# 959AI994/Multi-Gate-VAE

Measured on AMD Instinct MI355X. Metric: circuit-graphs/sec (train step), AIG-64k batch=64 per GPU, higher is better.
Workload: dtype f32 storage; dense products as bf16x3 split-precision MFMA, fp32 accumulate; 1 GPU; cfg2: DG_AE --type aig, 64 x 65536-node synthetic levelised DAGs per GPU (N=4194304, E=6558720, 120 levels), H=64, 4+4 rounds, layernorm, weights [1,4,4], negatives sampled; step includes the 7-scalar metrics copy (pinned, read one step behind); global_batch=64, parallelism=dp1

## Files before the change

### include/mgvae_hip.h

```cpp
#ifndef MGVAE_HIP_H
#define MGVAE_HIP_H
#include <stdint.h>
#ifdef __cplusplus
extern "C" {
#endif

#ifndef MGV_OK
#define MGV_OK 0
#define MGV_EINVAL (-1)
#define MGV_EUNSUPPORTED (-2)
#endif

int mgv_abi_version(void);

int mgv_struct_stage_fwd(int H, int64_t N, const float* h_in, const int32_t* nbr_ptr, const int32_t* nbr_idx,
                         const uint8_t* xcls, const float* xtab, int C, const float* Wc, const float* bc,
                         const float* Whh, const float* bhh, const float* ln_w, const float* ln_b, float ln_eps,
                         float* h_out, void* stream);
int mgv_struct_stage_bwd(int H, int64_t N, const float* h_in, const int32_t* nbr_ptr, const int32_t* nbr_idx,
                         const uint8_t* xcls, const float* xtab, int C, const float* Wc, const float* WcT,
                         const float* bc, const float* Whh, const float* WhhT, const float* bhh,
                         const float* ln_w, const float* ln_b, float ln_eps, const float* gy_direct,
                         const float* gy_agg, float* g_direct_out, float* g_agg_out, float* dWc, float* dbc,
                         float* dWhh, float* dbhh, float* dxtab, float* dln_w, float* dln_b, void* stream);
// ... 104 lines not shown
                          const float* gh, const float* h_prev, float* d_gh, float* g_hprev, void* stream);

int mgv_attn_pool_fwd(int W, int64_t N, const int32_t* in_ptr, const int32_t* in_src, const float* x, const float* u,
                      float* zbar, float* mstat, float* inv, void* stream);
int mgv_attn_pool_bwd(int W, int64_t N, const int32_t* in_ptr, const int32_t* in_src, const float* x, const float* u,
                      const float* zbar, const float* mstat, const float* inv, const float* dzbar, float* dx, float* du,
                      void* stream);

int mgv_sweep_pull_heavy(int H, int K, const int32_t* nodes, const int32_t* node_seg_ptr, int S, const int32_t* seg_e0,
                         const int32_t* seg_e1, const int32_t* out_dst, const int32_t* out_slot, const uint8_t* gslot,
                         const float* alpha, const float* dsc, const float* dzb, const float* attn_u, float* partial_ws,
                         float* ghs, void* stream);

int mgv_edge_dot_fwd(int H, int64_t E, const float* s, const float* t, int ld, const int64_t* src,
                     const int64_t* dst, int sigmoid, float* out, void* stream);
int mgv_edge_dot_bwd(int H, int64_t E, const float* s, const float* t, int ld, const int64_t* src,
                     const int64_t* dst, int sigmoid, const float* gout, float* ds, float* dt, void* stream);
int mgv_recon_loss_fwd(int H, const float* s, const float* t, int ld, const int64_t* pos_src, const int64_t* pos_dst,
                       int64_t Epos, const int64_t* neg_src, const int64_t* neg_dst, int64_t Eneg,
                       double* sums, uint64_t* counts, int32_t* pred_bin, double* workspace, int64_t workspace_doubles,
                       void* stream);
int mgv_recon_loss_bwd(int H, int64_t N, const float* s, const float* t, int ld, const int64_t* pos_src, const int64_t* pos_dst,
                       int64_t Epos, const int32_t* pos_out_ptr, const int32_t* pos_out_dst, const int32_t* pos_in_ptr,
                       const int32_t* pos_in_src, const int64_t* neg_src, const int64_t* neg_dst, int64_t Eneg,
                       const float* gscale, float* ds, float* dt, void* stream);
int mgv_recon_loss_bwd_csr(int H, int64_t N, const float* s, const float* t, int ld, const int32_t* pos_out_ptr,
                           const int32_t* pos_out_dst, const int32_t* pos_in_ptr, const int32_t* pos_in_src, int64_t Epos,
                           const int32_t* neg_out_ptr, const int32_t* neg_out_dst, const int32_t* neg_in_ptr,
                           const int32_t* neg_in_src, int64_t Eneg, const float* gscale, float* ds, float* dt,
                           int skip_pos_longer_than , void* stream);
int mgv_recon_heavy_lists(int H, const float* s, const float* t, int ld, int64_t Epos, const float* gscale, int K,
                          const int32_t* nodes, const int32_t* node_seg_ptr, int S, const int32_t* seg_node, const int32_t* seg_e0,
                          const int32_t* seg_e1, const int32_t* list, int which, float* partial_ws, float* out, void* stream);
int mgv_link_keys(int H, const float* s, const float* t, int ld, const int64_t* pos_src, const int64_t* pos_dst, int64_t P,
                  const int64_t* neg_src, const int64_t* neg_dst, int64_t Q, uint32_t* keys, float* scores, int32_t* status,
                  void* stream);
int mgv_link_rank_work_ints(int64_t n);
int mgv_link_rank(int64_t n, int64_t P, const uint32_t* sorted_keys, const int32_t* order, double* out, int32_t* work,
                  int64_t work_ints, void* stream);
int mgv_neg_sample(int64_t N, int64_t E, uint64_t seed, const int32_t* pos_out_ptr, const int32_t* pos_out_dst,
                   int64_t* neg_src, int64_t* neg_dst, int32_t* cnt_out, int32_t* cnt_in, int32_t* rank_out, int32_t* rank_in,
                   void* stream);
int mgv_neg_bucket(int64_t E, const int64_t* neg_src, const int64_t* neg_dst, const int32_t* out_ptr, const int32_t* in_ptr,
                   const int32_t* rank_out, const int32_t* rank_in, int64_t* srt_src, int64_t* srt_dst, int32_t* out_dst, int32_t* in_src,
                   void* stream);

int mgv_func_loss_fwd(int H, int64_t P, const float* hf, const int64_t* pair_a, const int64_t* pair_b,
                      const float* tt, float eps, float* dis, double* ws, double* workspace, int64_t workspace_doubles,
                      void* stream);
int mgv_func_loss_bwd_csr(int H, int64_t N, int64_t P, const float* hf, const int64_t* pair_a, const int64_t* pair_b, const float* tt_sim,
                          const float* dis, float eps, const double* workspace8, const float* grad_loss, const int32_t* a_ptr,
                          const int32_t* a_pair, const int32_t* b_ptr, const int32_t* b_pair, const float* add, float* dhf, void* stream);
int mgv_func_loss_bwd(int H, int64_t P, const float* hf, const int64_t* pair_a, const int64_t* pair_b,
                      const float* tt, const float* dis, float eps, const double* ws, const float* gscale,
                      float* dhf, void* stream);

int mgv_reparam_fwd(int64_t n, const float* mu, const float* logstd, const float* eps, uint64_t seed,
                    float* eps_out, float* z, double* klsum, void* stream);
int mgv_reparam_bwd(int64_t n, const float* mu, const float* logstd, const float* eps, const float* gz,
                    const float* gkl, float klcoef, float* dmu, float* dlogstd, void* stream);
int mgv_confusion(int64_t n, const int32_t* pred_bin, const int32_t* gt_bin, uint64_t* counts, void* stream);

int mgv_sum_workspace_doubles(void);
int mgv_colstats(int64_t N, int C, const float* Y, int ld, double* sums, double* workspace, int64_t workspace_doubles, void* stream);
int mgv_bn_act_fwd(int64_t N, int C, const float* Y, const float* mean, const float* invstd, const float* gamma,
                   const float* beta, float p_drop, uint64_t seed, float* A, void* stream);
// ... 87 lines not shown
```

### multi-gate-vae_amd/csrc/losses.hip

```cpp
#include "mgv_common.h"
#include "mgv_slab.h"
#include "../../include/mgvae_hip.h"

namespace mgv {

__device__ __forceinline__ void atomic_add4(float* p, const float4& v) {
    atomicAdd(p + 0, v.x); atomicAdd(p + 1, v.y); atomicAdd(p + 2, v.z); atomicAdd(p + 3, v.w);
}

__device__ __forceinline__ double block_sum_d(double v, double* red) {
    const int tid = threadIdx.x;
    __syncthreads();
    red[tid] = v;
    __syncthreads();
    for (int s = kThreads / 2; s > 0; s >>= 1) {
        if (tid < s) red[tid] += red[tid + s];
        __syncthreads();
    }
    return red[0];
}

template <int H, bool BWD>
__global__ __launch_bounds__(kThreads) void k_edge_dot(int64_t E, const float* s, const float* t, int ld,
                                                       const int64_t* src, const int64_t* dst, int sigmoid,
// ... 50 lines not shown
        if (ok) {
            u = pos ? a.psrc[e] : a.nsrc[e - a.Ep];
            v = pos ? a.pdst[e] : a.ndst[e - a.Ep];
            x = ld4(a.s + u * a.ld + 4 * lr);
            y = ld4(a.t + v * a.ld + 4 * lr);
        }
        const float val = group_sum<LPR>(dot4(x, y));
        const float p = sigmoidf_(val);
        if (!BWD) {
            if (ok && lr == 0) {
                const bool hit = p > 0.5f;
                if (pos) { lp -= logf(p + 1e-15f); tp += hit; fn += !hit; }
                else     { ln -= logf((1.0f - p) + 1e-15f); fp += hit; tn += !hit; }
                if (a.pred_bin) a.pred_bin[e] = hit ? 1 : 0;
            }
        } else if (ok) {
            const float dp = p * (1.0f - p);
            const float c = pos ? -wpos * dp / (p + 1e-15f) : wneg * dp / ((1.0f - p) + 1e-15f);
            atomic_add4(a.ds + u * a.ld + 4 * lr, scale4(c, y));
            atomic_add4(a.dt + v * a.ld + 4 * lr, scale4(c, x));
        }
    }
    if (!BWD) {
        const double sp = block_sum_d((double)lp, red);
        const double sn = block_sum_d((double)ln, red);
        const double c0 = block_sum_d((double)tp, red), c1 = block_sum_d((double)fp, red);
        const double c2 = block_sum_d((double)tn, red), c3 = block_sum_d((double)fn, red);
        if (threadIdx.x == 0) {
            a.slab[2 * blockIdx.x + 0] = sp; a.slab[2 * blockIdx.x + 1] = sn;
            atomicAdd(a.cnt + 0, (unsigned long long)c0); atomicAdd(a.cnt + 1, (unsigned long long)c1);
            atomicAdd(a.cnt + 2, (unsigned long long)c2); atomicAdd(a.cnt + 3, (unsigned long long)c3);
        }
    }
}

template <int H>
__global__ __launch_bounds__(kThreads) void k_recon_bwd_pull(int64_t N, const float* s, const float* t, int ld,
                                                             const int32_t* out_ptr, const int32_t* out_dst,
                                                             const int32_t* in_ptr, const int32_t* in_src, int64_t Ep,
                                                             const float* gscale, float* ds, float* dt) {
    constexpr int LPR = H / 4, RPB = kThreads / LPR;
    const int lr = threadIdx.x % LPR, slot = threadIdx.x / LPR;
    const float w = -(*gscale) / (float)Ep;
    for (int64_t n0 = (int64_t)blockIdx.x * RPB; n0 < N; n0 += (int64_t)gridDim.x * RPB) {
        const int64_t u = n0 + slot;
        if (u >= N) continue;
        const float4 su = ld4(s + u * ld + 4 * lr), tu = ld4(t + u * ld + 4 * lr);
        float4 gs = zero4(), gt = zero4();
        for (int e = out_ptr[u]; e < out_ptr[u + 1]; ++e) {
            const float4 tv = ld4(t + (int64_t)out_dst[e] * ld + 4 * lr);
            const float p = sigmoidf_(group_sum<LPR>(dot4(su, tv)));
            gs = fma4(w * p * (1.0f - p) / (p + 1e-15f), tv, gs);
        }
        for (int e = in_ptr[u]; e < in_ptr[u + 1]; ++e) {
            const float4 sv = ld4(s + (int64_t)in_src[e] * ld + 4 * lr);
            const float p = sigmoidf_(group_sum<LPR>(dot4(sv, tu)));
            gt = fma4(w * p * (1.0f - p) / (p + 1e-15f), sv, gt);
        }
        float* pds = ds + u * ld + 4 * lr;
        float* pdt = dt + u * ld + 4 * lr;
        st4(pds, add4(ld4(pds), gs));
        st4(pdt, add4(ld4(pdt), gt));
    }
}

template <int H>
// ... 281 lines not shown
        dmu[i] = g + gk * (-2.0f * m);
        dls[i] = g * eps[i] * sd + gk * (2.0f - 2.0f * sd * sd);
    }
}

__global__ __launch_bounds__(kThreads) void k_confusion(int64_t n, const int32_t* pred, const int32_t* gt, unsigned long long* cnt) {
    __shared__ double red[kThreads];
    unsigned int tp = 0, fp = 0, tn = 0, fn = 0;
    for (int64_t i = (int64_t)blockIdx.x * kThreads + threadIdx.x; i < n; i += (int64_t)gridDim.x * kThreads) {
        const int p = pred[i], g = gt[i];
        tp += (p == 1) & (g == 1); fp += (p == 1) & (g == 0); tn += (p == 0) & (g == 0); fn += (p == 0) & (g == 1);
    }
    const double c0 = block_sum_d((double)tp, red), c1 = block_sum_d((double)fp, red);
    const double c2 = block_sum_d((double)tn, red), c3 = block_sum_d((double)fn, red);
    if (threadIdx.x == 0) {
        atomicAdd(cnt + 0, (unsigned long long)c0); atomicAdd(cnt + 1, (unsigned long long)c1);
        atomicAdd(cnt + 2, (unsigned long long)c2); atomicAdd(cnt + 3, (unsigned long long)c3);
    }
}

inline int items_grid(int64_t items, int per_block) { return grid_for((items + per_block - 1) / per_block, 8); }

}

#define MGV_DISPATCH_H(H, CALL)                      \
    switch (H) {                                     \
        case 16: { constexpr int HH = 16; CALL; } break;  \
        case 32: { constexpr int HH = 32; CALL; } break;  \
        case 64: { constexpr int HH = 64; CALL; } break;  \
        case 128: { constexpr int HH = 128; CALL; } break; \
        default: return MGV_EUNSUPPORTED;            \
    }

extern "C" int mgv_edge_dot_fwd(int H, int64_t E, const float* s, const float* t, int ld, const int64_t* src,
                                const int64_t* dst, int sigmoid, float* out, void* stream) {
    MGV_CHECK_ARG(E >= 0 && s && t && out && ld >= H && ld % 4 == 0);
    if (E == 0) return MGV_OK;
    MGV_CHECK_ARG(src && dst);
    hipStream_t st = static_cast<hipStream_t>(stream);
    MGV_DISPATCH_H(H, hipLaunchKernelGGL((mgv::k_edge_dot<HH, false>), dim3(mgv::items_grid(E, mgv::kThreads / (HH / 4))), dim3(mgv::kThreads), 0, st,
                                         E, s, t, ld, src, dst, sigmoid, out, nullptr, nullptr, nullptr));
    MGV_LAUNCH_RET();
}

extern "C" int mgv_edge_dot_bwd(int H, int64_t E, const float* s, const float* t, int ld, const int64_t* src,
                                const int64_t* dst, int sigmoid, const float* gout, float* ds, float* dt, void* stream) {
    MGV_CHECK_ARG(E >= 0 && s && t && gout && ds && dt && ld >= H && ld % 4 == 0);
    if (E == 0) return MGV_OK;
    MGV_CHECK_ARG(src && dst);
    hipStream_t st = static_cast<hipStream_t>(stream);
    MGV_DISPATCH_H(H, hipLaunchKernelGGL((mgv::k_edge_dot<HH, true>), dim3(mgv::items_grid(E, mgv::kThreads / (HH / 4))), dim3(mgv::kThreads), 0, st,
                                         E, s, t, ld, src, dst, sigmoid, nullptr, gout, ds, dt));
    MGV_LAUNCH_RET();
}

extern "C" int mgv_recon_loss_fwd(int H, const float* s, const float* t, int ld, const int64_t* pos_src, const int64_t* pos_dst,
                                  int64_t Epos, const int64_t* neg_src, const int64_t* neg_dst, int64_t Eneg,
                                  double* sums, uint64_t* counts, int32_t* pred_bin, double* workspace, int64_t workspace_doubles,
                                  void* stream) {
    MGV_CHECK_ARG(s && t && sums && counts && Epos >= 0 && Eneg >= 0 && ld >= H && ld % 4 == 0);
    MGV_CHECK_ARG((Epos == 0 || (pos_src && pos_dst)) && (Eneg == 0 || (neg_src && neg_dst)));
    if (Epos + Eneg == 0) return MGV_OK;
    mgv::ReconArgs a{};
    a.s = s; a.t = t; a.ld = ld; a.psrc = pos_src; a.pdst = pos_dst; a.Ep = Epos; a.nsrc = neg_src; a.ndst = neg_dst; a.En = Eneg;
    a.sums = sums; a.cnt = reinterpret_cast<unsigned long long*>(counts); a.pred_bin = pred_bin;
    hipStream_t st = static_cast<hipStream_t>(stream);
    int grid = 0;
    MGV_DISPATCH_H(H, grid = mgv::items_grid(Epos + Eneg, mgv::kThreads / (HH / 4)));
    MGV_CHECK_ARG(workspace && workspace_doubles >= 2 * (int64_t)grid);
    a.slab = workspace;
    MGV_DISPATCH_H(H, hipLaunchKernelGGL((mgv::k_recon<HH, false>), dim3(grid), dim3(mgv::kThreads), 0, st, a));
    mgv::launch_slab_sum<double, double>(workspace, grid, 2, 2, sums, st);
    MGV_LAUNCH_RET();
}

extern "C" int mgv_recon_loss_bwd(int H, int64_t N, const float* s, const float* t, int ld, const int64_t* pos_src, const int64_t* pos_dst,
                                  int64_t Epos, const int32_t* pos_out_ptr, const int32_t* pos_out_dst, const int32_t* pos_in_ptr,
                                  const int32_t* pos_in_src, const int64_t* neg_src, const int64_t* neg_dst, int64_t Eneg,
                                  const float* gscale, float* ds, float* dt, void* stream) {
    MGV_CHECK_ARG(s && t && gscale && ds && dt && Epos >= 0 && Eneg >= 0 && N >= 0 && ld >= H && ld % 4 == 0);
    MGV_CHECK_ARG((Epos == 0 || (pos_src && pos_dst)) && (Eneg == 0 || (neg_src && neg_dst)));
    const bool pull = pos_out_ptr != nullptr;
    MGV_CHECK_ARG(!pull || (pos_in_ptr && (Epos == 0 || (pos_out_dst && pos_in_src))));
    if (H != 16 && H != 32 && H != 64) return MGV_EUNSUPPORTED;
    hipStream_t st = static_cast<hipStream_t>(stream);
    if (Epos > 0 && pull) {
        MGV_DISPATCH_H(H, hipLaunchKernelGGL((mgv::k_recon_bwd_pull<HH>), dim3(mgv::items_grid(N, mgv::kThreads / (HH / 4))), dim3(mgv::kThreads), 0, st,
                                             N, s, t, ld, pos_out_ptr, pos_out_dst, pos_in_ptr, pos_in_src, Epos, gscale, ds, dt));
    }
    for (int neg = (Epos > 0 && pull) ? 1 : 0; neg < 2; ++neg) {
        const int64_t E = neg ? Eneg : Epos;
        if (E == 0) continue;
        const int64_t* es = neg ? neg_src : pos_src;
        const int64_t* ed = neg ? neg_dst : pos_dst;
        const float wsc = 1.0f / (float)E;
        switch (H) {
            case 16: hipLaunchKernelGGL((mgv::k_recon_bwd_rows<16>), dim3(mgv::items_grid(E, mgv::kThreads / 16)), dim3(mgv::kThreads), 0, st, E, s, t, ld, es, ed, neg, wsc, gscale, ds, dt); break;
            case 32: hipLaunchKernelGGL((mgv::k_recon_bwd_rows<32>), dim3(mgv::items_grid(E, mgv::kThreads / 32)), dim3(mgv::kThreads), 0, st, E, s, t, ld, es, ed, neg, wsc, gscale, ds, dt); break;
            case 64: hipLaunchKernelGGL((mgv::k_recon_bwd_rows<64>), dim3(mgv::items_grid(E, mgv::kThreads / 64)), dim3(mgv::kThreads), 0, st, E, s, t, ld, es, ed, neg, wsc, gscale, ds, dt); break;
            default: return MGV_EUNSUPPORTED;
        }
    }
    MGV_LAUNCH_RET();
}

// ... 101 lines not shown
```

### multi-gate-vae_amd/csrc/neg_sample.hip

```cpp
#include "mgv_common.h"
#include "../../include/mgvae_hip.h"

namespace mgv {

__device__ __forceinline__ uint64_t splitmix64(uint64_t x) {
    x += 0x9E3779B97F4A7C15ull;
    x = (x ^ (x >> 30)) * 0xBF58476D1CE4E5B9ull;
    x = (x ^ (x >> 27)) * 0x94D049BB133111EBull;
    return x ^ (x >> 31);
}

__global__ __launch_bounds__(kThreads) void k_neg_sample(int64_t N, int64_t E, uint64_t seed, const int32_t* out_ptr, const int32_t* out_dst,
                                                        int64_t* neg_src, int64_t* neg_dst, int32_t* cnt_out, int32_t* cnt_in,
                                                        int32_t* rank_out, int32_t* rank_in) {
    for (int64_t i = (int64_t)blockIdx.x * kThreads + threadIdx.x; i < E; i += (int64_t)gridDim.x * kThreads) {
        uint64_t ctr = seed ^ ((uint64_t)i * 0xD1342543DE82EF95ull);
        int s, d;
        for (int attempt = 0;; ++attempt) {
            const uint64_t r = splitmix64(ctr + attempt);
            s = (int)(((r >> 32) * (uint64_t)N) >> 32);
            d = (int)(((r & 0xFFFFFFFFull) * (uint64_t)N) >> 32);
            bool ok = s != d;
            if (ok)
                for (int e = out_ptr[s]; e < out_ptr[s + 1]; ++e)
                    if (out_dst[e] == d) { ok = false; break; }
            if (ok || attempt >= 64) break;
        }
        neg_src[i] = s; neg_dst[i] = d;
        rank_out[i] = atomicAdd(cnt_out + s, 1);
        rank_in[i] = atomicAdd(cnt_in + d, 1);
    }
}

__global__ __launch_bounds__(kThreads) void k_neg_bucket(int64_t E, const int64_t* neg_src, const int64_t* neg_dst, const int32_t* out_ptr,
                                                        const int32_t* in_ptr, const int32_t* rank_out, const int32_t* rank_in, int64_t* srt_src,
                                                        int64_t* srt_dst, int32_t* out_dst, int32_t* in_src) {
    for (int64_t i = (int64_t)blockIdx.x * kThreads + threadIdx.x; i < E; i += (int64_t)gridDim.x * kThreads) {
        const int s = (int)neg_src[i], d = (int)neg_dst[i];
        const int p = out_ptr[s] + rank_out[i];
        srt_src[p] = s; srt_dst[p] = d; out_dst[p] = d;
        in_src[in_ptr[d] + rank_in[i]] = s;
    }
}

}

extern "C" int mgv_neg_sample(int64_t N, int64_t E, uint64_t seed, const int32_t* pos_out_ptr, const int32_t* pos_out_dst,
                              int64_t* neg_src, int64_t* neg_dst, int32_t* cnt_out, int32_t* cnt_in, int32_t* rank_out, int32_t* rank_in,
                              void* stream) {
    MGV_CHECK_ARG(N >= 2 && N < (1ll << 31) && E >= 0 && pos_out_ptr && neg_src && neg_dst && cnt_out && cnt_in && rank_out && rank_in);
    if (E == 0) return MGV_OK;
    hipLaunchKernelGGL(mgv::k_neg_sample, dim3(mgv::grid_for((E + mgv::kThreads - 1) / mgv::kThreads, 16)), dim3(mgv::kThreads), 0,
                       static_cast<hipStream_t>(stream), N, E, seed, pos_out_ptr, pos_out_dst, neg_src, neg_dst, cnt_out, cnt_in, rank_out, rank_in);
    MGV_LAUNCH_RET();
}

extern "C" int mgv_neg_bucket(int64_t E, const int64_t* neg_src, const int64_t* neg_dst, const int32_t* out_ptr, const int32_t* in_ptr,
                              const int32_t* rank_out, const int32_t* rank_in, int64_t* srt_src, int64_t* srt_dst, int32_t* out_dst, int32_t* in_src,
                              void* stream) {
    MGV_CHECK_ARG(E >= 0 && out_ptr && in_ptr && rank_out && rank_in);
    if (E == 0) return MGV_OK;
    MGV_CHECK_ARG(neg_src && neg_dst && srt_src && srt_dst && out_dst && in_src);
    hipLaunchKernelGGL(mgv::k_neg_bucket, dim3(mgv::grid_for((E + mgv::kThreads - 1) / mgv::kThreads, 16)), dim3(mgv::kThreads), 0,
                       static_cast<hipStream_t>(stream), E, neg_src, neg_dst, out_ptr, in_ptr, rank_out, rank_in, srt_src, srt_dst, out_dst, in_src);
    MGV_LAUNCH_RET();
}
```

### multi-gate-vae_amd/deepgate/_model_base.py

```python
import os

import torch
from torch import nn

from . import ops
from .arch.mlp import MLP
from .arch.tfmlp import TFMlpAggr
from .data import plan_of
from .digae_layer import DirectedInnerProductDecoder
from .sampling import NegativeEdges, negative_sampling, negative_sampling_device

EPS = 1e-15
DEVICE_SAMPLER = True
MAX_LOGSTD = 10


class FunctionalModel(nn.Module):
    ENCODER_ATTR = 'struct_encoder'
    GATES = ()

    def __init__(self, struct_encoder, num_rounds=1, dim_hidden=128, enable_encode=True, enable_reverse=True):
        super().__init__()
        setattr(self, self.ENCODER_ATTR, struct_encoder)
        self.decoder = DirectedInnerProductDecoder()
# ... 57 lines not shown
        return self.readout_prob(hf, clamp01=True, seed=seed)

    def _draw_negatives(self, hs, pos_edge_index, plan, edge_keys=None):
        if plan is not None and hs.is_cuda and hs.shape[0] >= 2 and DEVICE_SAMPLER:
            return negative_sampling_device(plan)
        return negative_sampling(pos_edge_index, hs.shape[0], keys=edge_keys)

    def link_metrics(self, hs, pos_edge_index, neg_edge_index=None, plan=None):
        with torch.no_grad():
            st = ops.linear(hs.detach(), self.hs_decompose.weight, self.hs_decompose.bias)
            if plan is not None and (plan.E != pos_edge_index.shape[1] or plan.N != hs.shape[0]):
                plan = None
            if neg_edge_index is None:
                neg_edge_index = self._draw_negatives(hs, pos_edge_index, plan)
            return ops.link_record(st, None, pos_edge_index, neg_edge_index)

    def recon_loss(self, hs, pos_edge_index, neg_edge_index=None, want_pred=True, edge_keys=None, plan=None, pass_hs=False, want_rank=False):
        if pass_hs and hs.requires_grad:
            st, self._hs_pass = ops.linear_passthrough(hs, self.hs_decompose.weight, self.hs_decompose.bias)
        else:
            st = ops.linear(hs, self.hs_decompose.weight, self.hs_decompose.bias)
        if plan is not None and (plan.E != pos_edge_index.shape[1] or plan.N != hs.shape[0]):
            plan = None
        neg_csr = None
        if neg_edge_index is None:
            neg_edge_index = self._draw_negatives(hs, pos_edge_index, plan, edge_keys)
        if plan is not None and hs.is_cuda and torch.is_tensor(neg_edge_index) and neg_edge_index.shape[1] > 0:
            cache = getattr(plan, '_neg_cache', None)
            key = (neg_edge_index.data_ptr(), neg_edge_index._version, tuple(neg_edge_index.shape), hs.shape[0])
            if cache is None or cache[0] is not neg_edge_index or cache[1] != key:
                from .sampling import bucket_negatives
                cache = plan._neg_cache = (neg_edge_index, key, bucket_negatives(neg_edge_index.long(), hs.shape[0]))
            neg_edge_index = cache[2]
        if isinstance(neg_edge_index, NegativeEdges):
            neg_csr, neg_edge_index = neg_edge_index.csr, neg_edge_index.edge_index
        loss, counts, pred_bin = ops.ReconLossFn.apply(st, pos_edge_index, neg_edge_index, want_pred, plan, neg_csr)
        self.last_confusion = counts
        self.last_link_metrics = ops.link_record(st, None, pos_edge_index, neg_edge_index) if want_rank else None
        Ep, En = pos_edge_index.shape[1], neg_edge_index.shape[1]
        gt_bin = None
        if want_pred:
            gt_bin = torch.zeros(Ep + En, dtype=torch.int32, device=hs.device)
            gt_bin[:Ep] = 1
        return loss, pred_bin if want_pred else None, gt_bin

    def load(self, model_path):
        checkpoint = torch.load(model_path, map_location=lambda storage, loc: storage)
        src = checkpoint['state_dict']
        state = {}
        for k, v in src.items():
            state[k[7:] if k.startswith('module') and not k.startswith('module_list') else k] = v
        own = self.state_dict()
        for k in list(state):
            if k in own:
                if state[k].shape != own[k].shape:
                    print('Skip loading parameter {}, required shape{}, loaded shape{}.'.format(k, own[k].shape, state[k].shape))
                    state[k] = own[k]
            else:
                print('Drop parameter {}.'.format(k))
        for k in own:
            if k not in state:
                print('No param {}.'.format(k))
                state[k] = own[k]
        self.load_state_dict(state, strict=False)

    def load_pretrained(self, pretrained_model_path=''):
        if pretrained_model_path == '':
            pretrained_model_path = os.path.join(os.path.dirname(__file__), 'pretrained', 'model.pth')
        self.load(pretrained_model_path)
```

### multi-gate-vae_amd/deepgate/ops.py

```python
import torch

from . import _hip
from ._hip import HipLibraryError, check, ptr

import os

F32 = torch.float32
I32 = torch.int32
U8 = torch.uint8
LN_EPS = 1e-5

PRECISION = os.environ.get('MGV_PRECISION', 'x3')
FIRST_STAGE_TABLE = True


def use_x3(H):
    return PRECISION == 'x3' and H in (32, 64)


def split_bf16(w):
    hi = w.to(torch.bfloat16)
    lo = (w - hi.to(torch.float32)).to(torch.bfloat16)
    return hi, lo

# ... 791 lines not shown
    @staticmethod
    def forward(ctx, s, t, edge_index, sigmoid):
        sd, td = check(s.detach().contiguous(), F32, 's'), check(t.detach().contiguous(), F32, 't')
        src, dst = _edge_rows(edge_index)
        E, H = src.numel(), sd.shape[1]
        out = torch.empty(E, dtype=F32, device=sd.device)
        _hip.call('mgv_edge_dot_fwd', H, E, ptr(sd), ptr(td), H, ptr(src), ptr(dst), int(bool(sigmoid)), ptr(out))
        ctx.save_for_backward(sd, td, src, dst)
        ctx.sigmoid = bool(sigmoid)
        return out

    @staticmethod
    def backward(ctx, gout):
        sd, td, src, dst = ctx.saved_tensors
        H = sd.shape[1]
        ds, dt = torch.zeros_like(sd), torch.zeros_like(td)
        gout = gout.contiguous()
        _hip.call('mgv_edge_dot_bwd', H, src.numel(), ptr(sd), ptr(td), H, ptr(src), ptr(dst), int(ctx.sigmoid),
                  ptr(gout), ptr(ds), ptr(dt))
        return ds, dt, None, None


def edge_dot(s, t, edge_index, sigmoid=True):
    return EdgeDotFn.apply(s, t, edge_index, sigmoid)


def dense_scores(s, t):
    M = t.shape[0]
    if M not in (16, 32, 64, 128):
        raise NotImplementedError('forward_all is only provided for 16/32/64/128 target rows')
    return linear(s, t.contiguous(), None)


class ReconLossFn(torch.autograd.Function):

    @staticmethod
    def forward(ctx, st, pos_edge_index, neg_edge_index, want_pred, plan=None, neg_csr=None):
        std = check(st.detach().contiguous(), F32, 'st')
        N, H2 = std.shape
        H = H2 // 2
        ps, pd = _edge_rows(pos_edge_index)
        ns, nd = _edge_rows(neg_edge_index)
        Ep, En = ps.numel(), ns.numel()
        dev = std.device
        sums = torch.zeros(2, dtype=torch.float64, device=dev)
        counts = torch.zeros(4, dtype=torch.int64, device=dev)
        pred = torch.empty(Ep + En, dtype=torch.int32, device=dev) if want_pred else None
        t_view = std[:, H:]
        _hip.call('mgv_recon_loss_fwd', H, ptr(std), ptr(t_view), H2, ptr(ps), ptr(pd), Ep, ptr(ns), ptr(nd), En,
                  ptr(sums), ptr(counts), ptr(pred), *_sw(std.device))
        loss = (sums[0] / max(Ep, 1) + sums[1] / max(En, 1)).to(F32)
        ctx.save_for_backward(std, ps, pd, ns, nd)
        ctx.plan, ctx.neg_csr = plan, neg_csr
        ctx.mark_non_differentiable(counts)
        if pred is not None:
            ctx.mark_non_differentiable(pred)
            return loss, counts, pred
        return loss, counts, torch.empty(0, dtype=torch.int32, device=dev)

    @staticmethod
    def backward(ctx, gloss, _gc, _gp):
        global _SWEEP_BWD_EVENT
        if _SWEEP_BWD_EVENT is not None and gloss.is_cuda:
            torch.cuda.current_stream().wait_event(_SWEEP_BWD_EVENT)
            _SWEEP_BWD_EVENT = None
        std, ps, pd, ns, nd = ctx.saved_tensors
        H2 = std.shape[1]
        H = H2 // 2
        g = gloss.detach().to(F32).reshape(1).contiguous()
        pl = ctx.plan
        if pl is not None and ctx.neg_csr is not None:
            dst_ = torch.empty_like(std)
            heavy = [(0, pl.heavy_segments(True), pl.out_dst), (1, pl.heavy_segments(False), pl.in_src)]
            skip = pl.HEAVY_ROW if any(hv is not None for _, hv, _ in heavy) else 0
            _hip.call('mgv_recon_loss_bwd_csr', H, std.shape[0], ptr(std), ptr(std[:, H:]), H2, ptr(pl.out_ptr), ptr(pl.out_dst),
                      ptr(pl.in_ptr), ptr(pl.in_src), ps.numel(), *[ptr(c) for c in ctx.neg_csr], ns.numel(), ptr(g), ptr(dst_),
                      ptr(dst_[:, H:]), skip)
            for which, hv, lst in heavy:
                if hv is not None:
                    pw = workspace(hv['S'] * H, std.device)
                    _hip.call('mgv_recon_heavy_lists', H, ptr(std), ptr(std[:, H:]), H2, ps.numel(), ptr(g), hv['K'], ptr(hv['nodes']),
                              ptr(hv['node_seg_ptr']), hv['S'], ptr(hv['seg_node']), ptr(hv['seg_e0']), ptr(hv['seg_e1']), ptr(lst), which,
                              ptr(pw), ptr(dst_[:, H:]) if which else ptr(dst_))
            return dst_, None, None, None, None, None
        dst_ = torch.zeros_like(std)
        csr = (pl.out_ptr, pl.out_dst, pl.in_ptr, pl.in_src) if pl is not None else (None, None, None, None)
        _hip.call('mgv_recon_loss_bwd', H, std.shape[0], ptr(std), ptr(std[:, H:]), H2, ptr(ps), ptr(pd), ps.numel(),
                  *[ptr(c) for c in csr], ptr(ns), ptr(nd), ns.numel(), ptr(g), ptr(dst_), ptr(dst_[:, H:]))
        return dst_, None, None, None, None, None


def confusion_counts(pred_bin, gt_bin):
    counts = torch.zeros(4, dtype=torch.int64, device=pred_bin.device)
    _hip.call('mgv_confusion', pred_bin.numel(), ptr(check(pred_bin.contiguous(), torch.int32, 'pred_bin')),
              ptr(check(gt_bin.contiguous(), torch.int32, 'gt_bin')), ptr(counts))
    return counts


LINK_RECORD_WORDS = 8


def link_record(st_or_s, t=None, pos_edge_index=None, neg_edge_index=None, return_scores=False):
    neg = getattr(neg_edge_index, 'edge_index', neg_edge_index)
    P, Q = int(pos_edge_index.shape[1]), int(neg.shape[1])
    if P == 0 or Q == 0:
        raise ValueError('Only one class present (%d positive, %d negative pairs): ROC-AUC and average precision are not defined' % (P, Q))
    sd = check(st_or_s.detach().contiguous(), F32, 'st' if t is None else 's')
    if t is None:
        ld = sd.shape[1]
        H = ld // 2
        td = sd[:, H:]
    else:
        td = check(t.detach().contiguous(), F32, 't')
        ld = H = sd.shape[1]
        if td.shape != sd.shape:
            raise HipLibraryError('s and t must have the same shape (got %s and %s)' % (tuple(sd.shape), tuple(td.shape)))
    n = P + Q
    if n >= 1 << 31:
        raise HipLibraryError('mgv_link_keys failed: %s (%d pairs; the ranking holds fewer than 2^31)' % (_hip._ERR[-2], n))
    ps, pd = _edge_rows(pos_edge_index)
    ns, nd = _edge_rows(neg)
# ... 284 lines not shown
```

### multi-gate-vae_amd/deepgate/sampling.py

```python
import itertools

import torch

from . import _hip
from ._hip import ptr

_CALLS = itertools.count()


class NegativeEdges:

    def __init__(self, edge_index, out_ptr, out_dst, in_ptr, in_src):
        self.edge_index, self.out_ptr, self.out_dst, self.in_ptr, self.in_src = edge_index, out_ptr, out_dst, in_ptr, in_src

    @property
    def csr(self):
        return self.out_ptr, self.out_dst, self.in_ptr, self.in_src


def bucket_negatives(neg, N):
    dev = neg.device
    E = int(neg.shape[1])
    i32 = dict(dtype=torch.int32, device=dev)
    src, dst = neg[0].contiguous(), neg[1].contiguous()
    in_ptr, out_ptr = torch.empty(N + 1, **i32), torch.empty(N + 1, **i32)
    in_src, in_dst, out_dst, out_slot = (torch.empty(max(E, 1), **i32) for _ in range(4))
    n_s = _hip.call_value('mgv_plan_csr_scratch_ints', N, E)
    scratch = torch.empty(n_s, **i32)
    status = torch.empty(2, **i32)
    _hip.call('mgv_plan_csr', N, E, ptr(src), ptr(dst), ptr(in_ptr), ptr(in_src), ptr(in_dst), ptr(out_ptr), ptr(out_dst), ptr(out_slot),
              None, None, ptr(scratch), n_s, ptr(status))
    if int(status[0].item()) != 0:
        raise ValueError('neg_edge_index holds node ids outside [0, num_nodes)')
    counts = (out_ptr[1:] - out_ptr[:-1]).long()
    srt_src = torch.repeat_interleave(torch.arange(N, device=dev), counts, output_size=E)
    srt = torch.stack([srt_src, out_dst[:E].long()])
    return NegativeEdges(srt, out_ptr, out_dst, in_ptr, in_src)


def negative_sampling_device(plan, num_neg_samples=None, generator=None):
    N, dev = plan.N, plan.device
    if getattr(plan, 'num_self_loops', None) is None:
        plan.count_self_loops()
    E = (plan.E - plan.num_self_loops) + N if num_neg_samples is None else int(num_neg_samples)
    base = generator.initial_seed() if generator is not None else torch.initial_seed()
    seed = (base * 0x9E3779B97F4A7C15 + next(_CALLS) * 0xD1B54A32D192ED03 + 0x2545F4914F6CDD1D) & 0xFFFFFFFFFFFFFFFF
    scratch = torch.zeros(2, N, dtype=torch.int32, device=dev)
    neg = torch.empty(2, E, dtype=torch.int64, device=dev)
    rank = torch.empty(2, max(E, 1), dtype=torch.int32, device=dev)
    _hip.call('mgv_neg_sample', N, E, seed, ptr(plan.out_ptr), ptr(plan.out_dst), ptr(neg[0]), ptr(neg[1]), ptr(scratch[0]), ptr(scratch[1]),
              ptr(rank[0]), ptr(rank[1]))
    ptrs = torch.zeros(2, N + 1, dtype=torch.int32, device=dev)
    for k in range(2):
        ptrs[k, 1:] = torch.cumsum(scratch[k], 0, dtype=torch.int32)
    srt = torch.empty(2, E, dtype=torch.int64, device=dev)
    out_dst = torch.empty(max(E, 1), dtype=torch.int32, device=dev)
    in_src = torch.empty(max(E, 1), dtype=torch.int32, device=dev)
    _hip.call('mgv_neg_bucket', E, ptr(neg[0]), ptr(neg[1]), ptr(ptrs[0]), ptr(ptrs[1]), ptr(rank[0]), ptr(rank[1]),
              ptr(srt[0]), ptr(srt[1]), ptr(out_dst), ptr(in_src))
    ss = torch.empty(N + 1 + E, dtype=torch.int32, device=dev)
    _hip.call('mgv_sort_lists_i32', N, E, ptr(ptrs[0]), ptr(out_dst), ptr(ss), ss.numel())
    _hip.call('mgv_sort_lists_i32', N, E, ptr(ptrs[1]), ptr(in_src), ptr(ss), ss.numel())
    srt[1].copy_(out_dst[:E])
    return NegativeEdges(srt, ptrs[0], out_dst, ptrs[1], in_src)


def sorted_edge_keys(pos_edge_index, num_nodes):
    src, dst = pos_edge_index[0].long(), pos_edge_index[1].long()
    keep = src != dst
    return torch.sort(src[keep] * int(num_nodes) + dst[keep]).values


def negative_sampling(pos_edge_index, num_nodes, num_neg_samples=None, generator=None, keys=None):
    dev = pos_edge_index.device
    N = int(num_nodes)
    if keys is None:
        keys = sorted_edge_keys(pos_edge_index, N)
    want = int(keys.numel()) + N if num_neg_samples is None else int(num_neg_samples)
    out = torch.empty((2, 0), dtype=torch.long, device=dev)
    guard = 0
    while out.shape[1] < want:
        m = want - out.shape[1]
        m = m + m // 8 + 16
        s = torch.randint(0, N, (m,), device=dev, generator=generator)
        d = torch.randint(0, N, (m,), device=dev, generator=generator)
        k = s * N + d
        ok = s != d
        if keys.numel() > 0:
            pos = torch.searchsorted(keys, k).clamp_(max=keys.numel() - 1)
            ok &= keys[pos] != k
        out = torch.cat([out, torch.stack([s[ok], d[ok]])], dim=1)
        guard += 1
        if guard > 64:
            raise RuntimeError('negative_sampling: graph too dense to draw %d non-edges' % want)
    return out[:, :want].contiguous()
```

Before: 991.7 graphs/s.

## Compute recon loss forward from CSR and skip materializing negative pair lists

Adds a CSR-driven forward recon-loss kernel that walks each source node's positive and negative out-lists, loads the source row once and prefetches partner indices. Heavy rows get a separate segment kernel. Negative sampling no longer writes int64 sorted src/dst pair arrays; they are built lazily only when edge_index is requested (prediction or ranking paths). This removes the int64 edge-pair traffic and the separate pair construction, at the cost of more code paths and reliance on the heavy-segment split for load balance.

```diff
diff --git a/include/mgvae_hip.h b/include/mgvae_hip.h
--- a/include/mgvae_hip.h
+++ b/include/mgvae_hip.h
@@ -160,6 +160,13 @@
 int mgv_recon_heavy_lists(int H, const float* s, const float* t, int ld, int64_t Epos, const float* gscale, int K,
                           const int32_t* nodes, const int32_t* node_seg_ptr, int S, const int32_t* seg_node, const int32_t* seg_e0,
                           const int32_t* seg_e1, const int32_t* list, int which, float* partial_ws, float* out, void* stream);
+int mgv_recon_loss_fwd_csr(int H, int64_t N, const float* s, const float* t, int ld, const int32_t* pos_out_ptr,
+                           const int32_t* pos_out_dst, int64_t Epos, const int32_t* neg_out_ptr, const int32_t* neg_out_dst,
+                           int64_t Eneg, double* sums, uint64_t* counts, double* workspace, int64_t workspace_doubles,
+                           int skip_pos_longer_than, void* stream);
+int mgv_recon_heavy_lists_fwd(int H, const float* s, const float* t, int ld, int K, const int32_t* nodes, int S,
+                              const int32_t* seg_node, const int32_t* seg_e0, const int32_t* seg_e1, const int32_t* list,
+                              double* sums, uint64_t* counts, double* workspace, int64_t workspace_doubles, void* stream);
 int mgv_link_keys(int H, const float* s, const float* t, int ld, const int64_t* pos_src, const int64_t* pos_dst, int64_t P,
                   const int64_t* neg_src, const int64_t* neg_dst, int64_t Q, uint32_t* keys, float* scores, int32_t* status,
                   void* stream);
diff --git a/multi-gate-vae_amd/csrc/losses.hip b/multi-gate-vae_amd/csrc/losses.hip
--- a/multi-gate-vae_amd/csrc/losses.hip
+++ b/multi-gate-vae_amd/csrc/losses.hip
@@ -106,6 +106,101 @@
             atomicAdd(a.cnt + 2, (unsigned long long)c2); atomicAdd(a.cnt + 3, (unsigned long long)c3);
         }
     }
+}
+
+template <int H>
+__global__ __launch_bounds__(kThreads) void k_recon_fwd_csr(int64_t N, const float* s, const float* t, int ld, const int32_t* pout_ptr,
+                                                            const int32_t* pout_dst, int64_t Ep, const int32_t* nout_ptr,
+                                                            const int32_t* nout_dst, int64_t En, unsigned long long* cnt, double* slab,
+                                                            int skip_len) {
+    constexpr int LPR = H / 4, RPB = kThreads / LPR, K = 4;
+    __shared__ double red[kThreads];
+    const int lr = threadIdx.x % LPR, slot = threadIdx.x / LPR;
+    int64_t first, end, stride;
+    if ((gridDim.x & 7) == 0) {
+        const int64_t chunk = ((N + 8 * RPB - 1) / (8 * RPB)) * RPB;
+        first = (blockIdx.x & 7) * chunk + (int64_t)(blockIdx.x >> 3) * RPB;
+        end = min(N, ((blockIdx.x & 7) + 1) * chunk);
+        stride = (int64_t)(gridDim.x >> 3) * RPB;
+    } else {
+        first = (int64_t)blockIdx.x * RPB; end = N; stride = (int64_t)gridDim.x * RPB;
+    }
+    double lp = 0.0, ln = 0.0;
+    unsigned int tp = 0, fp = 0, tn = 0, fn = 0;
+    for (int64_t n0 = first; n0 < end; n0 += stride) {
+        const int64_t u = n0 + slot;
+        if (u >= end) continue;
+        const float4 su = ld4(s + u * ld + 4 * lr);
+        int b0 = 0, b1 = 0, c0 = 0, c1 = 0;
+        if (Ep > 0) {
+            b0 = pout_ptr[u]; c0 = pout_ptr[u + 1] - b0;
+            if (skip_len > 0 && c0 > skip_len) c0 = 0;
+        }
+        if (En > 0) { b1 = nout_ptr[u]; c1 = nout_ptr[u + 1] - b1; }
+        c1 += c0;
+        auto partner = [&](int j) -> int { return j < c0 ? pout_dst[b0 + j] : nout_dst[b1 + (j - c0)]; };
+        int id[K];
+#pragma unroll
+        for (int k = 0; k < K; ++k) id[k] = k < c1 ? partner(k) : 0;
+        for (int j0 = 0; j0 < c1; j0 += K) {
+            float4 v[K];
+#pragma unroll
+            for (int k = 0; k < K; ++k)
+                if (j0 + k < c1) v[k] = ld4(t + (int64_t)id[k] * ld + 4 * lr);
+            int nid[K];
+#pragma unroll
+            for (int k = 0; k < K; ++k) nid[k] = j0 + K + k < c1 ? partner(j0 + K + k) : 0;
+#pragma unroll
+            for (int k = 0; k < K; ++k) {
+                const int j = j0 + k;
+                if (j < c1) {
+                    const float p = sigmoidf_(group_sum<LPR>(dot4(su, v[k])));
+                    const bool hit = p > 0.5f;
+                    if (j < c0) { lp -= (double)logf(p + 1e-15f); tp += hit; fn += !hit; }
+                    else        { ln -= (double)logf((1.0f - p) + 1e-15f); fp += hit; tn += !hit; }
+                }
+            }
+#pragma unroll
+            for (int k = 0; k < K; ++k) id[k] = nid[k];
+        }
+    }
+    if (lr != 0) { lp = 0.0; ln = 0.0; tp = 0; fp = 0; tn = 0; fn = 0; }
+    const double sp = block_sum_d(lp, red);
+    const double sn = block_sum_d(ln, red);
+    const double c0 = block_sum_d((double)tp, red), c1 = block_sum_d((double)fp, red);
+    const double c2 = block_sum_d((double)tn, red), c3 = block_sum_d((double)fn, red);
+    if (threadIdx.x == 0) {
+        slab[2 * blockIdx.x + 0] = sp; slab[2 * blockIdx.x + 1] = sn;
+        if (c0 + c1 + c2 + c3 > 0) {
+            atomicAdd(cnt + 0, (unsigned long long)c0); atomicAdd(cnt + 1, (unsigned long long)c1);
+            atomicAdd(cnt + 2, (unsigned long long)c2); atomicAdd(cnt + 3, (unsigned long long)c3);
+        }
+    }
+}
+
+template <int H>
+__global__ __launch_bounds__(kThreads) void k_recon_heavy_seg_fwd(int S, const int32_t* seg_node, const int32_t* seg_e0, const int32_t* seg_e1,
+                                                                  const int32_t* nodes, const float* s, const float* t, int ld,
+                                                                  const int32_t* list, unsigned long long* cnt, double* slab) {
+    constexpr int LPR = H / 4, G = kThreads / LPR;
+    __shared__ double red[kThreads];
+    const int lr = threadIdx.x % LPR, grp = threadIdx.x / LPR;
+    unsigned int tp = 0, fn = 0;
+    for (int sg = blockIdx.x; sg < S; sg += gridDim.x) {
+        const int64_t u = nodes[seg_node[sg]];
+        const float4 own = ld4(s + u * ld + 4 * lr);
+        double lp = 0.0;
+        for (int e = seg_e0[sg] + grp; e < seg_e1[sg]; e += G) {
+            const float4 v = ld4(t + (int64_t)list[e] * ld + 4 * lr);
+            const float p = sigmoidf_(group_sum<LPR>(dot4(own, v)));
+            const bool hit = p > 0.5f;
+            lp -= (double)logf(p + 1e-15f); tp += hit; fn += !hit;
+        }
+        const double sp = block_sum_d(lr == 0 ? lp : 0.0, red);
+        if (threadIdx.x == 0) slab[sg] = sp;
+    }
+    const double c0 = block_sum_d(lr == 0 ? (double)tp : 0.0, red), c3 = block_sum_d(lr == 0 ? (double)fn : 0.0, red);
+    if (threadIdx.x == 0) { atomicAdd(cnt + 0, (unsigned long long)c0); atomicAdd(cnt + 3, (unsigned long long)c3); }
 }
 
 template <int H>
@@ -453,6 +548,14 @@
         default: return MGV_EUNSUPPORTED;            \
     }
 
+#define MGV_DISPATCH_H64(H, CALL)                    \
+    switch (H) {                                     \
+        case 16: { constexpr int HH = 16; CALL; } break;  \
+        case 32: { constexpr int HH = 32; CALL; } break;  \
+        case 64: { constexpr int HH = 64; CALL; } break;  \
+        default: return MGV_EUNSUPPORTED;            \
+    }
+
 extern "C" int mgv_edge_dot_fwd(int H, int64_t E, const float* s, const float* t, int ld, const int64_t* src,
                                 const int64_t* dst, int sigmoid, float* out, void* stream) {
     MGV_CHECK_ARG(E >= 0 && s && t && out && ld >= H && ld % 4 == 0);
@@ -492,6 +595,38 @@
     a.slab = workspace;
     MGV_DISPATCH_H(H, hipLaunchKernelGGL((mgv::k_recon<HH, false>), dim3(grid), dim3(mgv::kThreads), 0, st, a));
     mgv::launch_slab_sum<double, double>(workspace, grid, 2, 2, sums, st);
+    MGV_LAUNCH_RET();
+}
+
+extern "C" int mgv_recon_loss_fwd_csr(int H, int64_t N, const float* s, const float* t, int ld, const int32_t* pos_out_ptr,
+                                      const int32_t* pos_out_dst, int64_t Epos, const int32_t* neg_out_ptr, const int32_t* neg_out_dst,
+                                      int64_t Eneg, double* sums, uint64_t* counts, double* workspace, int64_t workspace_doubles,
+                                      int skip_pos_longer_than, void* stream) {
+    MGV_CHECK_ARG(s && t && sums && counts && Epos >= 0 && Eneg >= 0 && N >= 0 && N < (1ll << 31) && ld >= H && ld % 4 == 0 && skip_pos_longer_than >= 0);
+    MGV_CHECK_ARG((Epos == 0 || (pos_out_ptr && pos_out_dst)) && (Eneg == 0 || (neg_out_ptr && neg_out_dst)));
+    if (H != 16 && H != 32 && H != 64) return MGV_EUNSUPPORTED;
+    if (N == 0 || Epos + Eneg == 0) return MGV_OK;
+    hipStream_t st = static_cast<hipStream_t>(stream);
+    const int grid = mgv::items_grid(N, mgv::kThreads / (H / 4));
+    MGV_CHECK_ARG(workspace && workspace_doubles >= 2 * (int64_t)grid);
+    auto* cnt = reinterpret_cast<unsigned long long*>(counts);
+    MGV_DISPATCH_H64(H, hipLaunchKernelGGL((mgv::k_recon_fwd_csr<HH>), dim3(grid), dim3(mgv::kThreads), 0, st, N, s, t, ld, pos_out_ptr, pos_out_dst,
+                                         Epos, neg_out_ptr, neg_out_dst, Eneg, cnt, workspace, skip_pos_longer_than));
+    mgv::launch_slab_sum<double, double>(workspace, grid, 2, 2, sums, st);
+    MGV_LAUNCH_RET();
+}
+
+extern "C" int mgv_recon_heavy_lists_fwd(int H, const float* s, const float* t, int ld, int K, const int32_t* nodes, int S,
+                                         const int32_t* seg_node, const int32_t* seg_e0, const int32_t* seg_e1, const int32_t* list,
+                                         double* sums, uint64_t* counts, double* workspace, int64_t workspace_doubles, void* stream) {
+    MGV_CHECK_ARG(K >= 0 && S >= 0 && s && t && sums && counts && ld >= H && ld % 4 == 0);
+    if (H != 16 && H != 32 && H != 64) return MGV_EUNSUPPORTED;
+    if (K == 0 || S == 0) return MGV_OK;
+    MGV_CHECK_ARG(nodes && seg_node && seg_e0 && seg_e1 && list && workspace && workspace_doubles >= S);
+    hipStream_t st = static_cast<hipStream_t>(stream);
+    MGV_DISPATCH_H64(H, hipLaunchKernelGGL((mgv::k_recon_heavy_seg_fwd<HH>), dim3(S < 4096 ? S : 4096), dim3(mgv::kThreads), 0, st, S, seg_node, seg_e0,
+                                         seg_e1, nodes, s, t, ld, list, reinterpret_cast<unsigned long long*>(counts), workspace));
+    mgv::launch_slab_sum<double, double>(workspace, S, 1, 1, sums, st);
     MGV_LAUNCH_RET();
 }
 
diff --git a/multi-gate-vae_amd/csrc/neg_sample.hip b/multi-gate-vae_amd/csrc/neg_sample.hip
--- a/multi-gate-vae_amd/csrc/neg_sample.hip
+++ b/multi-gate-vae_amd/csrc/neg_sample.hip
@@ -32,13 +32,15 @@
     }
 }
 
+template <bool PAIRS>
 __global__ __launch_bounds__(kThreads) void k_neg_bucket(int64_t E, const int64_t* neg_src, const int64_t* neg_dst, const int32_t* out_ptr,
                                                         const int32_t* in_ptr, const int32_t* rank_out, const int32_t* rank_in, int64_t* srt_src,
                                                         int64_t* srt_dst, int32_t* out_dst, int32_t* in_src) {
     for (int64_t i = (int64_t)blockIdx.x * kThreads + threadIdx.x; i < E; i += (int64_t)gridDim.x * kThreads) {
         const int s = (int)neg_src[i], d = (int)neg_dst[i];
         const int p = out_ptr[s] + rank_out[i];
-        srt_src[p] = s; srt_dst[p] = d; out_dst[p] = d;
+        if (PAIRS) { srt_src[p] = s; srt_dst[p] = d; }
+        out_dst[p] = d;
         in_src[in_ptr[d] + rank_in[i]] = s;
     }
 }
@@ -60,8 +62,13 @@
                               void* stream) {
     MGV_CHECK_ARG(E >= 0 && out_ptr && in_ptr && rank_out && rank_in);
     if (E == 0) return MGV_OK;
-    MGV_CHECK_ARG(neg_src && neg_dst && srt_src && srt_dst && out_dst && in_src);
-    hipLaunchKernelGGL(mgv::k_neg_bucket, dim3(mgv::grid_for((E + mgv::kThreads - 1) / mgv::kThreads, 16)), dim3(mgv::kThreads), 0,
-                       static_cast<hipStream_t>(stream), E, neg_src, neg_dst, out_ptr, in_ptr, rank_out, rank_in, srt_src, srt_dst, out_dst, in_src);
+    MGV_CHECK_ARG(neg_src && neg_dst && out_dst && in_src && (srt_src == nullptr) == (srt_dst == nullptr));
+    const dim3 grid(mgv::grid_for((E + mgv::kThreads - 1) / mgv::kThreads, 16));
+    if (srt_src)
+        hipLaunchKernelGGL(mgv::k_neg_bucket<true>, grid, dim3(mgv::kThreads), 0, static_cast<hipStream_t>(stream), E, neg_src, neg_dst, out_ptr, in_ptr,
+                           rank_out, rank_in, srt_src, srt_dst, out_dst, in_src);
+    else
+        hipLaunchKernelGGL(mgv::k_neg_bucket<false>, grid, dim3(mgv::kThreads), 0, static_cast<hipStream_t>(stream), E, neg_src, neg_dst, out_ptr, in_ptr,
+                           rank_out, rank_in, nullptr, nullptr, out_dst, in_src);
     MGV_LAUNCH_RET();
 }
diff --git a/multi-gate-vae_amd/deepgate/_model_base.py b/multi-gate-vae_amd/deepgate/_model_base.py
--- a/multi-gate-vae_amd/deepgate/_model_base.py
+++ b/multi-gate-vae_amd/deepgate/_model_base.py
@@ -113,12 +113,16 @@
                 from .sampling import bucket_negatives
                 cache = plan._neg_cache = (neg_edge_index, key, bucket_negatives(neg_edge_index.long(), hs.shape[0]))
             neg_edge_index = cache[2]
+        En = None
         if isinstance(neg_edge_index, NegativeEdges):
-            neg_csr, neg_edge_index = neg_edge_index.csr, neg_edge_index.edge_index
+            neg, neg_csr, En = neg_edge_index, neg_edge_index.csr, neg_edge_index.num_edges
+            neg_edge_index = En if ops.recon_csr_forward(st, want_pred, plan, neg_csr) and not want_rank else neg.edge_index
         loss, counts, pred_bin = ops.ReconLossFn.apply(st, pos_edge_index, neg_edge_index, want_pred, plan, neg_csr)
         self.last_confusion = counts
         self.last_link_metrics = ops.link_record(st, None, pos_edge_index, neg_edge_index) if want_rank else None
-        Ep, En = pos_edge_index.shape[1], neg_edge_index.shape[1]
+        Ep = pos_edge_index.shape[1]
+        if En is None:
+            En = neg_edge_index.shape[1]
         gt_bin = None
         if want_pred:
             gt_bin = torch.zeros(Ep + En, dtype=torch.int32, device=hs.device)
diff --git a/multi-gate-vae_amd/deepgate/ops.py b/multi-gate-vae_amd/deepgate/ops.py
--- a/multi-gate-vae_amd/deepgate/ops.py
+++ b/multi-gate-vae_amd/deepgate/ops.py
@@ -847,6 +847,10 @@
     return linear(s, t.contiguous(), None)
 
 
+def recon_csr_forward(st, want_pred, plan, neg_csr):
+    return plan is not None and neg_csr is not None and not want_pred and st.is_cuda and st.shape[1] // 2 in (16, 32, 64)
+
+
 class ReconLossFn(torch.autograd.Function):
 
     @staticmethod
@@ -854,18 +858,36 @@
         std = check(st.detach().contiguous(), F32, 'st')
         N, H2 = std.shape
         H = H2 // 2
+        dev = std.device
+        sums = torch.zeros(2, dtype=torch.float64, device=dev)
+        counts = torch.zeros(4, dtype=torch.int64, device=dev)
+        t_view = std[:, H:]
+        if recon_csr_forward(std, want_pred, plan, neg_csr):
+            Ep = int(pos_edge_index.shape[1])
+            En = int(neg_edge_index) if isinstance(neg_edge_index, int) else int(neg_edge_index.shape[1])
+            hv = plan.heavy_segments(True)
+            wsd = sum_ws(dev) if hv is None else workspace(max(hv['S'], sum_ws(dev).numel()), dev, torch.float64)
+            _hip.call('mgv_recon_loss_fwd_csr', H, N, ptr(std), ptr(t_view), H2, ptr(plan.out_ptr), ptr(plan.out_dst), Ep,
+                      ptr(neg_csr[0]), ptr(neg_csr[1]), En, ptr(sums), ptr(counts), ptr(wsd), wsd.numel(),
+                      plan.HEAVY_ROW if hv is not None else 0)
+            if hv is not None and Ep > 0:
+                _hip.call('mgv_recon_heavy_lists_fwd', H, ptr(std), ptr(t_view), H2, hv['K'], ptr(hv['nodes']), hv['S'], ptr(hv['seg_node']),
+                          ptr(hv['seg_e0']), ptr(hv['seg_e1']), ptr(plan.out_dst), ptr(sums), ptr(counts), ptr(wsd), wsd.numel())
+            ctx.save_for_backward(std)
+            ctx.Ep, ctx.En = Ep, En
+            ctx.plan, ctx.neg_csr = plan, neg_csr
+            loss = (sums[0] / max(Ep, 1) + sums[1] / max(En, 1)).to(F32)
+            ctx.mark_non_differentiable(counts)
+            return loss, counts, torch.empty(0, dtype=torch.int32, device=dev)
         ps, pd = _edge_rows(pos_edge_index)
         ns, nd = _edge_rows(neg_edge_index)
         Ep, En = ps.numel(), ns.numel()
-        dev = std.device
-        sums = torch.zeros(2, dtype=torch.float64, device=dev)
-        counts = torch.zeros(4, dtype=torch.int64, device=dev)
         pred = torch.empty(Ep + En, dtype=torch.int32, device=dev) if want_pred else None
-        t_view = std[:, H:]
         _hip.call('mgv_recon_loss_fwd', H, ptr(std), ptr(t_view), H2, ptr(ps), ptr(pd), Ep, ptr(ns), ptr(nd), En,
                   ptr(sums), ptr(counts), ptr(pred), *_sw(std.device))
         loss = (sums[0] / max(Ep, 1) + sums[1] / max(En, 1)).to(F32)
         ctx.save_for_backward(std, ps, pd, ns, nd)
+        ctx.Ep, ctx.En = Ep, En
         ctx.plan, ctx.neg_csr = plan, neg_csr
         ctx.mark_non_differentiable(counts)
         if pred is not None:
@@ -879,29 +901,31 @@
         if _SWEEP_BWD_EVENT is not None and gloss.is_cuda:
             torch.cuda.current_stream().wait_event(_SWEEP_BWD_EVENT)
             _SWEEP_BWD_EVENT = None
-        std, ps, pd, ns, nd = ctx.saved_tensors
+        std = ctx.saved_tensors[0]
         H2 = std.shape[1]
         H = H2 // 2
         g = gloss.detach().to(F32).reshape(1).contiguous()
         pl = ctx.plan
+        Ep, En = ctx.Ep, ctx.En
         if pl is not None and ctx.neg_csr is not None:
             dst_ = torch.empty_like(std)
             heavy = [(0, pl.heavy_segments(True), pl.out_dst), (1, pl.heavy_segments(False), pl.in_src)]
             skip = pl.HEAVY_ROW if any(hv is not None for _, hv, _ in heavy) else 0
             _hip.call('mgv_recon_loss_bwd_csr', H, std.shape[0], ptr(std), ptr(std[:, H:]), H2, ptr(pl.out_ptr), ptr(pl.out_dst),
-                      ptr(pl.in_ptr), ptr(pl.in_src), ps.numel(), *[ptr(c) for c in ctx.neg_csr], ns.numel(), ptr(g), ptr(dst_),
+                      ptr(pl.in_ptr), ptr(pl.in_src), Ep, *[ptr(c) for c in ctx.neg_csr], En, ptr(g), ptr(dst_),
                       ptr(dst_[:, H:]), skip)
             for which, hv, lst in heavy:
                 if hv is not None:
                     pw = workspace(hv['S'] * H, std.device)
-                    _hip.call('mgv_recon_heavy_lists', H, ptr(std), ptr(std[:, H:]), H2, ps.numel(), ptr(g), hv['K'], ptr(hv['nodes']),
+                    _hip.call('mgv_recon_heavy_lists', H, ptr(std), ptr(std[:, H:]), H2, Ep, ptr(g), hv['K'], ptr(hv['nodes']),
                               ptr(hv['node_seg_ptr']), hv['S'], ptr(hv['seg_node']), ptr(hv['seg_e0']), ptr(hv['seg_e1']), ptr(lst), which,
                               ptr(pw), ptr(dst_[:, H:]) if which else ptr(dst_))
             return dst_, None, None, None, None, None
+        _, ps, pd, ns, nd = ctx.saved_tensors
         dst_ = torch.zeros_like(std)
         csr = (pl.out_ptr, pl.out_dst, pl.in_ptr, pl.in_src) if pl is not None else (None, None, None, None)
-        _hip.call('mgv_recon_loss_bwd', H, std.shape[0], ptr(std), ptr(std[:, H:]), H2, ptr(ps), ptr(pd), ps.numel(),
-                  *[ptr(c) for c in csr], ptr(ns), ptr(nd), ns.numel(), ptr(g), ptr(dst_), ptr(dst_[:, H:]))
+        _hip.call('mgv_recon_loss_bwd', H, std.shape[0], ptr(std), ptr(std[:, H:]), H2, ptr(ps), ptr(pd), Ep,
+                  *[ptr(c) for c in csr], ptr(ns), ptr(nd), En, ptr(g), ptr(dst_), ptr(dst_[:, H:]))
         return dst_, None, None, None, None, None
 
 
diff --git a/multi-gate-vae_amd/deepgate/sampling.py b/multi-gate-vae_amd/deepgate/sampling.py
--- a/multi-gate-vae_amd/deepgate/sampling.py
+++ b/multi-gate-vae_amd/deepgate/sampling.py
@@ -8,10 +8,24 @@
 _CALLS = itertools.count()
 
 
+def pairs_by_source(out_ptr, out_dst, E):
+    N = int(out_ptr.numel()) - 1
+    counts = (out_ptr[1:] - out_ptr[:-1]).long()
+    src = torch.repeat_interleave(torch.arange(N, device=out_ptr.device), counts, output_size=E)
+    return torch.stack([src, out_dst[:E].long()])
+
+
 class NegativeEdges:
 
-    def __init__(self, edge_index, out_ptr, out_dst, in_ptr, in_src):
-        self.edge_index, self.out_ptr, self.out_dst, self.in_ptr, self.in_src = edge_index, out_ptr, out_dst, in_ptr, in_src
+    def __init__(self, edge_index, out_ptr, out_dst, in_ptr, in_src, num_edges=None):
+        self._edge_index, self.out_ptr, self.out_dst, self.in_ptr, self.in_src = edge_index, out_ptr, out_dst, in_ptr, in_src
+        self.num_edges = int(edge_index.shape[1]) if num_edges is None else int(num_edges)
+
+    @property
+    def edge_index(self):
+        if self._edge_index is None:
+            self._edge_index = pairs_by_source(self.out_ptr, self.out_dst, self.num_edges)
+        return self._edge_index
 
     @property
     def csr(self):
@@ -32,10 +46,7 @@
               None, None, ptr(scratch), n_s, ptr(status))
     if int(status[0].item()) != 0:
         raise ValueError('neg_edge_index holds node ids outside [0, num_nodes)')
-    counts = (out_ptr[1:] - out_ptr[:-1]).long()
-    srt_src = torch.repeat_interleave(torch.arange(N, device=dev), counts, output_size=E)
-    srt = torch.stack([srt_src, out_dst[:E].long()])
-    return NegativeEdges(srt, out_ptr, out_dst, in_ptr, in_src)
+    return NegativeEdges(pairs_by_source(out_ptr, out_dst, E), out_ptr, out_dst, in_ptr, in_src)
 
 
 def negative_sampling_device(plan, num_neg_samples=None, generator=None):
@@ -53,16 +64,14 @@
     ptrs = torch.zeros(2, N + 1, dtype=torch.int32, device=dev)
     for k in range(2):
         ptrs[k, 1:] = torch.cumsum(scratch[k], 0, dtype=torch.int32)
-    srt = torch.empty(2, E, dtype=torch.int64, device=dev)
     out_dst = torch.empty(max(E, 1), dtype=torch.int32, device=dev)
     in_src = torch.empty(max(E, 1), dtype=torch.int32, device=dev)
     _hip.call('mgv_neg_bucket', E, ptr(neg[0]), ptr(neg[1]), ptr(ptrs[0]), ptr(ptrs[1]), ptr(rank[0]), ptr(rank[1]),
-              ptr(srt[0]), ptr(srt[1]), ptr(out_dst), ptr(in_src))
+              None, None, ptr(out_dst), ptr(in_src))
     ss = torch.empty(N + 1 + E, dtype=torch.int32, device=dev)
     _hip.call('mgv_sort_lists_i32', N, E, ptr(ptrs[0]), ptr(out_dst), ptr(ss), ss.numel())
     _hip.call('mgv_sort_lists_i32', N, E, ptr(ptrs[1]), ptr(in_src), ptr(ss), ss.numel())
-    srt[1].copy_(out_dst[:E])
-    return NegativeEdges(srt, ptrs[0], out_dst, ptrs[1], in_src)
+    return NegativeEdges(None, ptrs[0], out_dst, ptrs[1], in_src, num_edges=E)
 
 
 def sorted_edge_keys(pos_edge_index, num_nodes):
```

Measured after the change: 995.5 graphs/s (median of 6 runs). No clear change (+0.4%).
